# VachaLab/gorder

Measured on AMD Instinct MI355X. Metric: trajectory frames/sec, higher is better.
Workload: dtype f32

## Files before the change

gorder_amd/csrc/gorder_hip.hip:

```cpp
#include <hip/hip_runtime.h>

#include <dlfcn.h>

#include <cmath>
#include <cstdio>
#include <cstdlib>
#include <cstring>
#include <mutex>
#include <new>
#include <string>
#include <deque>
#include <type_traits>
#include <vector>

#include "../../include/gorder_hip.h"
#include "gm_math.h"
#include "plan.h"
#include "collect_store.h"
#include "device_mem.h"
#include "replay_rows.h"
#include "timewise_blocks.h"
#include "ordermap_final.h"
#include "order_route.h"
#include "molecule_rows.h"
// ... 59 lines not shown

struct RepAcc {
    DBuf<u64> acc, rep;
    uint32_t n_rep = 1;
    size_t words = 0;
    bool alloc(size_t n_words, uint32_t n_rep_wanted) {
        words = n_words;
        n_rep = gorder::replica_count(n_rep_wanted, n_words);
        return acc.alloc(words) && rep.alloc((size_t)n_rep * words);
    }
    void reset() { acc.reset(); rep.reset(); words = 0; }
    hipError_t zero_async(hipStream_t stream) {
        const hipError_t e = hipMemsetAsync(acc, 0, words * sizeof(u64), stream);
        return e != hipSuccess ? e : hipMemsetAsync(rep, 0, (size_t)n_rep * words * sizeof(u64), stream);
    }
    hipError_t fold(hipStream_t stream) {
        hipLaunchKernelGGL(k_fold_replicas, dim3((uint32_t)((words + 255) / 256)), dim3(256), 0, stream, acc.get(), rep.get(), n_rep, (uint32_t)words);
        return hipGetLastError();
    }
};

struct gorder_hip_handle {
    void *traj_cache = nullptr;
    void (*traj_cache_free)(gorder_hip_handle *) = nullptr;
    Plan plan;
    gorder_tables_t tables{};
    int device = 0;
    Stream own_stream;
    hipStream_t stream = nullptr;
    DBuf<Tile> d_tiles;
    DBuf<Item> d_items;
    DBuf<uint32_t> d_tile_slots;
    DBuf<DirectItem> d_direct;
    DBuf<Tile> d_ua_tiles;
    DBuf<gorder::UaItem> d_ua_items;
    DBuf<uint32_t> d_ua_tile_slots;
    uint32_t map_nx = 0, map_ny = 0;
    DBuf<u64> d_map_sums, d_map_cnts;
    DBuf<u64> d_map_packed;
    DBuf<u64> d_map_rec;
    DBuf<gorder::MapRun> d_ua_runs, d_runs;
    DBuf<uint32_t> d_ua_run_begin, d_run_begin;
    DBuf<Item> d_items_by_slot;
    DBuf<uint32_t> d_ua_item_run, d_item_run;
    DBuf<uint4> d_lgrid;
    DBuf<LocalRowPre> d_lrowpre;
    DBuf<LocalEdge> d_ledge;
    DBuf<float4> d_lfinfo;
    static constexpr uint32_t kDecidePause = 16;
    DBuf<uint32_t> d_lsummary;
    HBuf<uint32_t> h_lsummary;
    Event lsummary_written;
    bool lsummary_pending = false;
    uint32_t decide_pause = 0;
    uint64_t decide_submits = 0, decide_paused_submits = 0;
    DBuf<uint32_t> d_lneed;
    DBuf<uint2> d_ltodo;
    size_t map_lds_bytes = 0;
    bool map_staged = false;
    uint64_t map_pending = 0;
    uint64_t map_fold_limit = kMapFoldLimit;
    uint32_t map_max_mol = 1;
    DBuf<u64> d_tw_sums, d_tw_cnts;
    uint64_t tw_cap = 0;
    DBuf<u64> d_twx_blocks, d_twx_rows, d_twx_totals, d_twx_edge;
    DBuf<uint32_t> d_twx_groups;
    DBuf<float> d_twx_out;
    DBuf<uint32_t> d_omx_groups;
    DBuf<float> d_omx_out;
    ExtraArgs extra{};
    DBuf<uint32_t> d_geom_group;
    DBuf<float> d_shapes;
    DBuf<float> d_inv_box;
    uint32_t dyn_slab = 4, local_slab = 4;
    bool local_halo = false;
    size_t local_rec_stride = 0;
    DBuf<XtcCheckpoint> d_xtc_cp;
    bool dyn = false;
    DBuf<uint32_t> d_dyn_cloud, d_dyn_heads;
    DBuf<uint32_t> d_dyn_cell_of, d_dyn_count;
    DBuf<float> d_dyn_rec;
    DBuf<float4> d_dyn_normals;
    DBuf<DynCov> d_dyn_cov;
    std::vector<float> last_normals;
    std::vector<float> manual_normals;
    uint32_t manual_frames = 0;
    bool manual_active = false;
    DBuf<uint32_t> d_err;
    u64 *d_acc = nullptr;
    DBuf<u64> own_acc;
    DBuf<u64> d_rep;
    uint32_t n_rep = 32;
    bool rep_dirty = false;
    size_t acc_words = 0;
    DBuf<uint32_t> d_heads, d_membrane, d_methyl_begin, d_methyl_atoms;
    DBuf<uint8_t> d_aflags;
    size_t aflags_rows = 0;
    DBuf<float> d_adist;
    DBuf<float> d_sph_spill, d_sph_stats;
    uint32_t sph_spill = 0, sph_slab = 1u << 20, sph_threads = 1024;
    DBuf<char> d_cl_scratch;
    DBuf<uint32_t> d_cl_head_slot;
    DBuf<uint8_t> d_cl_carry, d_cl_is0;
    DBuf<float> d_cl_stats;
    uint32_t cl_slab = 1, cl_m_max = 0;
    bool cl_stored_w = false;
    bool cl_have_carry = false;
    bool cl_cut = false;
    uint32_t cl_tiles = 0, cl_sort = 0;
    std::vector<uint8_t> cl_is0;
    DBuf<uint32_t> d_lcell_of, d_lcell_count, d_lcell_fill;
    DBuf<float> d_ltrig;
    DBuf<uint32_t> d_arow, d_aframes;
    std::vector<uint32_t> up_arow, up_aframes;
    bool up_arow_valid = false, up_aframes_valid = false;
    bool have_assignment = false;
    uint64_t assignment_frame = 0;
    bool spec_enabled = false;
    DBuf<uint2> d_own;
    DBuf<float4> d_mom;
    DBuf<float> d_head_z;
    DBuf<uint32_t> d_own_head_begin;
    DBuf<uint2> d_own_heads;
    DBuf<float> d_spec_center;
    DBuf<uint8_t> d_spec_ok;
    DBuf<uint32_t> d_spec_counters;
    static constexpr uint32_t kSpecRing = 8;
    HBuf<uint32_t> h_spec_counters;
    Event spec_counters_copied[kSpecRing];
    uint64_t spec_ring_frames[kSpecRing] = {};
    DBuf<uint32_t> d_spec_mol_begin;
    DBuf<SpecSample> d_spec_samples;
    uint64_t spec_batches = 0, spec_fixed = 0, spec_exact_frames = 0;
    DBuf<float> d_stage_xyz[2], d_stage_box[2];
    Event stage_copied[2], stage_computed[2];
    bool stage_used[2] = {false, false};
    int stage_next = 0;
    Stream copy_stream;
    float n2 = 1.0f, n2sq = 1.0f;
    int axis = -1;
    int frames_per_stage = kFramesPerStage;
    bool membrane_is_frame = false;
    bool use_gather = false;
    uint32_t wg_capacity = 256u * 6u;
    uint32_t wg_target = 0;
    uint32_t lw = 0;
    size_t lds_bytes = 0;
    uint64_t n_frames = 0;
    uint64_t err_index = 0;
    std::string err_msg;
    static constexpr uint32_t kTimingEvents = 1024;
    struct TimingSeg { uint32_t label, ev_a, ev_b; };
    bool timing_on = false;
    Event timing_ev[kTimingEvents];
    uint32_t timing_next_ev = 0;
    int timing_open_label = -1;
    uint32_t timing_open_ev = 0;
    std::deque<TimingSeg> timing_pending;
    std::vector<std::string> timing_labels;
    std::vector<double> timing_label_ms;
    std::vector<uint64_t> timing_label_n;
    uint64_t timing_launches = 0;
    std::string timed_kernels;
    std::vector<uint32_t> host_heads, host_dyn_heads;
    DBuf<uint32_t> d_mol_slot0;
    uint64_t err_frame = 0;
// ... 192 lines not shown
        size_t k = 0;
        while (k < h->timing_labels.size() && h->timing_labels[k] != label) k++;
        if (k == h->timing_labels.size()) {
            h->timing_labels.push_back(label);
            h->timing_label_ms.push_back(0.0);
            h->timing_label_n.push_back(0);
            if (!h->timed_kernels.empty()) h->timed_kernels += " + ";
            h->timed_kernels += label;
        }
        h->timing_open_label = (int)k;
        h->timing_open_ev = ev;
    }
    return GORDER_OK;
}
#define TIMING_MARK(h, label)                                   \
    do {                                                        \
        const int tm_ = timing_mark(h, label);                  \
        if (tm_ != GORDER_OK) return tm_;                       \
    } while (0)

bool env_flag(const char *name) {
    const char *v = getenv(name);
    return v && *v && strcmp(v, "0") != 0;
}

int fold_replicas(gorder_hip_handle *h) {
    if (!h->rep_dirty || !h->d_rep) return GORDER_OK;
    const uint32_t n = 4u * h->plan.n_acc;
    hipLaunchKernelGGL(k_fold_replicas, dim3((n + 255) / 256), dim3(256), 0, h->stream, h->d_acc, h->d_rep, h->n_rep, n);
    HIP_TRY(h, hipGetLastError());
    h->rep_dirty = false;
    return GORDER_OK;
}

int fold_maps(gorder_hip_handle *h) {
    if (!h->extra.maps || !h->map_pending) return GORDER_OK;
    const size_t n = (size_t)h->plan.n_acc * h->map_nx * h->map_ny;
    const uint32_t blocks = (uint32_t)std::min<size_t>((n + 255) / 256, 256 * 16);
    hipLaunchKernelGGL(k_fold_maps, dim3(blocks), dim3(256), 0, h->stream, h->d_map_packed, h->d_map_sums, h->d_map_cnts,
                       n, h->tables.leaflets.method != GORDER_LEAFLETS_NONE ? 1 : 0);
    HIP_TRY(h, hipGetLastError());
    h->map_pending = 0;
    return GORDER_OK;
}

int launch_cell_list(gorder_hip_handle *h, const LocalArgs &lo, uint32_t ns, uint32_t n_list, void *counts, size_t count_bytes) {
    const bool three = env_flag("GORDER_HIP_LOCAL_THREE_KERNELS");
    TIMING_MARK(h, n_list <= kLocalBuildMax && !three ? "k_local_build" : "k_local_bin + k_local_scan + k_local_scatter");
    if (n_list <= kLocalBuildMax && !three) {
        if (n_list <= 2u * 8192u) hipLaunchKernelGGL(k_local_build<2>, dim3(ns), dim3(1024), kLocalBuildLds, h->stream, lo);
        else if (n_list <= 5u * 8192u) hipLaunchKernelGGL(k_local_build<5>, dim3(ns), dim3(1024), kLocalBuildLds, h->stream, lo);
        else hipLaunchKernelGGL(k_local_build<kLocalBuildTrips>, dim3(ns), dim3(1024), kLocalBuildLds, h->stream, lo);
        return GORDER_OK;
    }
    HIP_TRY(h, hipMemsetAsync(counts, 0, count_bytes, h->stream));
    const dim3 ga((n_list + 255) / 256, ns);
    hipLaunchKernelGGL(k_local_bin, ga, dim3(256), 0, h->stream, lo);
    hipLaunchKernelGGL(k_local_scan, dim3(ns), dim3(1024), 0, h->stream, lo);
    hipLaunchKernelGGL(k_local_scatter, ga, dim3(256), 0, h->stream, lo);
    return GORDER_OK;
}

int run_dynamic_normals(gorder_hip_handle *h, const FrameArgs &a) {
    int st;
    const uint32_t n_mol = h->plan.n_mol_total;
    if ((st = ensure(h, h->d_dyn_normals, (size_t)a.n_frames * n_mol)) != GORDER_OK) return st;
    const gorder_dynamic_normal_t &dn = h->tables.dynamic_normal;
    const size_t ncell = (size_t)kLocalMaxCells1D * kLocalMaxCells1D;
    LocalArgs lo{};
    lo.xyz = a.xyz; lo.box9 = a.box9; lo.n_atoms = a.n_atoms;
    lo.n_mol_total = n_mol; lo.heads = h->d_dyn_heads; lo.membrane = h->d_dyn_cloud; lo.n_membrane = dn.n_cloud;
    lo.dim = 2; lo.pbc = a.pbc; lo.radius = dn.radius; lo.radius_thr = local_radius_threshold(dn.radius);
    lo.halo = 0; lo.rec_stride = dn.n_cloud;
    lo.cell_of = h->d_dyn_cell_of; lo.trig = h->d_dyn_rec;
    lo.cell_count = h->d_dyn_count; lo.cell_fill = h->d_dyn_count + h->dyn_slab * (ncell + 1);
    lo.err = h->d_err; lo.aframes = nullptr; lo.write_dist_frame = -1;
    for (uint32_t done = 0; done < a.n_frames; done += h->dyn_slab) {
        const uint32_t ns = std::min(a.n_frames - done, h->dyn_slab);
        lo.frame0 = done;
        lo.n_slab = ns;
        if ((st = launch_cell_list(h, lo, ns, dn.n_cloud, h->d_dyn_count,
                                   (size_t)h->dyn_slab * (2 * ncell + 1) * sizeof(uint32_t))) != GORDER_OK) return st;
        TIMING_MARK(h, "k_dyn_cov + k_dyn_eigen");
        hipLaunchKernelGGL(k_dyn_cov, dim3((n_mol + 15) / 16, ns), dim3(256), 0, h->stream, lo, h->d_dyn_cov);
        hipLaunchKernelGGL(k_dyn_eigen, dim3((uint32_t)(((size_t)ns * n_mol + 255) / 256)), dim3(256), 0, h->stream, lo, h->d_dyn_cov,
                           h->d_dyn_normals);
    }
    HIP_TRY(h, hipGetLastError());
    h->last_normals.resize(4 * (size_t)n_mol);
    HIP_TRY(h, hipMemcpyAsync(h->last_normals.data(), h->d_dyn_normals + (size_t)(a.n_frames - 1) * n_mol,
                              4 * sizeof(float) * (size_t)n_mol, hipMemcpyDeviceToHost, h->stream));
    return GORDER_OK;
}

template <int V, int... Vs, class F>
void with_int(int v, F &&f) {
    if constexpr (sizeof...(Vs) > 0) { if (v != V) return with_int<Vs...>(v, f); }
    f(std::integral_constant<int, V>{});
}
template <class F> void with_bool(bool v, F &&f) { if (v) f(std::true_type{}); else f(std::false_type{}); }
template <class F> void with_axis(int axis, F &&f) { with_int<2, 1, 0, -1>(axis, f); }
template <class F> void with_npf(int npf, F &&f) { with_int<4, 5>(npf, f); }
static_assert(gorder::kStageFrames == kRecFrames && gorder::kStageFrames == (uint32_t)kFramesPerStage, "order_route.h: frames of a stage");

int collect_copy_out(gorder_hip_handle *h, gorder::CollectStore &store, const void *d_block, const uint64_t *frames, size_t n_rows);
int launch_molecule_rows(gorder_hip_handle *h, const FrameArgs &a, const gorder::OrderRoute &route) {
    const Plan &p = h->plan;
    const uint32_t n_tiles = (uint32_t)p.tiles.size();
    const bool ac = (h->tables.flags & GORDER_FLAG_TRIG_ACOS_COS) != 0;
    const size_t wpf = (size_t)h->mol.n_groups * p.n_mol_total;
    const uint32_t sub = gorder::molecule_rows_subrange(a.n_frames, wpf, h->mol_stage_bytes);
    int st;
    if ((st = ensure(h, h->d_mol_stage, wpf * sub)) != GORDER_OK) return st;
    MolRowArgs mr{};
    mr.runs = h->d_mol_runs; mr.run_begin = h->d_mol_run_begin; mr.stage = h->d_mol_stage; mr.words_per_frame = (uint32_t)wpf;
    for (uint32_t lo = 0; lo < a.n_frames; lo += sub) {
        const uint32_t hi = std::min(a.n_frames, lo + sub), nf = hi - lo;
        const gorder::FrameChunks c = gorder::extras_chunks(nf, n_tiles, h->wg_target, h->wg_capacity, false, true);
        const uint64_t grid = (uint64_t)n_tiles * c.n_chunks;
        if (grid > 0x7fffffffull) return fail(h, GORDER_ERR_INVALID_ARGUMENT, "batch too large");
        FrameArgs b = a;
        b.frame0 = lo; b.n_frames = hi; b.frames_per_chunk = c.frames_per_chunk;
        TIMING_MARK(h, route.label);
        HIP_TRY(h, hipMemsetAsync(h->d_mol_stage, 0, wpf * nf * sizeof(unsigned long long), h->stream));
        const dim3 g((uint32_t)grid), blk(kBlock);
        with_npf(route.npf, [&](auto NPF) { with_bool(b.pbc, [&](auto PBC) { with_bool(b.leaflets, [&](auto LF) {
            if (ac)
                hipLaunchKernelGGL((k_bonds_tiled_mol<NPF(), true, PBC(), LF(), -1>), g, blk, h->lds_bytes, h->stream, b, mr, b.xyz, b.box9,
                                   b.aflags, b.arow, h->d_tiles, h->d_mol_items, h->d_tile_slots, n_tiles, h->lw);
            else with_int<2, -1>(h->axis, [&](auto AX) {
                hipLaunchKernelGGL((k_bonds_tiled_mol<NPF(), false, PBC(), LF(), AX()>), g, blk, h->lds_bytes, h->stream, b, mr, b.xyz, b.box9,
                                   b.aflags, b.arow, h->d_tiles, h->d_mol_items, h->d_tile_slots, n_tiles, h->lw);
            });
        }); }); });
        HIP_TRY(h, hipGetLastError());
        if ((st = collect_copy_out(h, h->mol_store, h->d_mol_stage, h->mol_frame_index + lo, nf)) != GORDER_OK) return st;
    }
    return GORDER_OK;
}

int launch_orders(gorder_hip_handle *h, FrameArgs &a, const gorder::OrderRoute &route) {
    using gorder::BondFamily, gorder::FrameChunks;
    const Plan &p = h->plan;
    const uint32_t n_tiles = (uint32_t)p.tiles.size();
    const bool ac = (h->tables.flags & GORDER_FLAG_TRIG_ACOS_COS) != 0;
    if (h->dyn && !h->manual_active) {
        ST_TRY(run_dynamic_normals(h, a));
    }
    if (h->extra.geom_kind) {
        int st2;
        if ((st2 = ensure(h, h->d_shapes, (size_t)a.n_frames * 8)) != GORDER_OK) return st2;
        const gorder_geometry_t &ge = h->tables.geometry;
        GeomArgs ga{};
        ga.xyz = a.xyz; ga.box9 = a.box9; ga.n_atoms = a.n_atoms; ga.pbc = a.pbc;
        ga.kind = ge.kind; ga.reference = ge.reference; ga.orientation = ge.orientation;
        for (int d = 0; d < 3; d++) { ga.point[d] = ge.point[d]; ga.structure_box[d] = ge.structure_box[d]; }
        for (int d = 0; d < 2; d++) { ga.xdim[d] = ge.xdim[d]; ga.ydim[d] = ge.ydim[d]; ga.zdim[d] = ge.zdim[d]; ga.span[d] = ge.span[d]; }
        ga.radius = ge.radius; ga.group = h->d_geom_group; ga.n_group = ge.n_group;
        ga.shapes = h->d_shapes; ga.err = h->d_err;
        TIMING_MARK(h, "k_geom_shapes");
        hipLaunchKernelGGL(k_geom_shapes, dim3(a.n_frames), dim3(256), 0, h->stream, ga);
        HIP_TRY(h, hipGetLastError());
    }
    if (route.family == BondFamily::Tiled || route.family == BondFamily::Gather) {
        const FrameChunks c = gorder::tiled_chunks(a.n_frames, (uint32_t)h->frames_per_stage, n_tiles, h->wg_target, h->wg_capacity);
        a.frames_per_chunk = c.frames_per_chunk;
        const uint64_t grid = (uint64_t)n_tiles * c.n_chunks;
        if (grid > 0x7fffffffull) return fail(h, GORDER_ERR_INVALID_ARGUMENT, "batch too large");
        const dim3 g((uint32_t)grid), b(kBlock);
// ... 503 lines not shown
    }
    e.maps = 1; e.plane = om.plane; e.x0 = om.span_x[0]; e.y0 = om.span_y[0];
    e.binx = om.bin[0]; e.biny = om.bin[1]; e.nx = h->map_nx; e.ny = h->map_ny;
    e.inv_binx = 1.0f / om.bin[0]; e.inv_biny = 1.0f / om.bin[1];
    e.bin_core = (om.bin[0] >= 0x1p-40f && om.bin[0] <= 0x1p+40f && om.bin[1] >= 0x1p-40f && om.bin[1] <= 0x1p+40f) ? 1 : 0;
    e.map_packed = h->d_map_packed;
    return GORDER_OK;
}

static int create_geometry(gorder_hip_handle *h, const gorder_tables_t *t) {
    const gorder_geometry_t &ge = t->geometry;
    if (ge.kind == GORDER_GEOM_NONE) return GORDER_OK;
    ExtraArgs &e = h->extra;
    if (ge.kind > GORDER_GEOM_SPHERE || ge.reference > GORDER_GEOMREF_GROUP || ge.orientation > 2)
        return fail(h, GORDER_ERR_INVALID_ARGUMENT, "geometry kind/reference/orientation");
    if (ge.reference == GORDER_GEOMREF_BOX_CENTER && !t->handle_pbc)
        return fail(h, GORDER_ERR_INVALID_ARGUMENT, "box-centre reference needs handle_pbc (pbc.rs:243-245)");
    if (ge.reference == GORDER_GEOMREF_POINT && t->handle_pbc &&
        !(ge.structure_box[0] > 0.0f && ge.structure_box[1] > 0.0f && ge.structure_box[2] > 0.0f))
        return fail(h, GORDER_ERR_INVALID_ARGUMENT, "geometry.structure_box");
    if (ge.reference == GORDER_GEOMREF_GROUP) {
        if (!ge.group || ge.n_group == 0) return fail(h, GORDER_ERR_INVALID_ARGUMENT, "geometry.group");
        std::vector<uint32_t> grp(ge.group, ge.group + ge.n_group);
        for (uint32_t a : grp)
            if (a >= t->n_atoms) return fail(h, GORDER_ERR_INVALID_ARGUMENT, "geometry group index out of range");
        ST_TRY(upload(h, h->d_geom_group, grp));
    }
    e.geom_kind = (int)ge.kind; e.geom_invert = ge.invert ? 1 : 0; e.geom_orient = (int)ge.orientation;
    e.geom_thr = local_radius_threshold(ge.radius);
    h->tables.geometry.group = nullptr;
    return GORDER_OK;
}

static int create_accumulators(gorder_hip_handle *h) {
    const Plan &p = h->plan;
    ST_TRY(allocate(h, h->d_err, kErrWords + 2u));
    HIP_TRY(h, hipMemset(h->d_err, 0xff, kErrWords * sizeof(uint32_t)));
    HIP_TRY(h, hipMemset(h->d_err + kErrWords, 0, 2u * sizeof(uint32_t)));
    h->acc_words = 4 * (size_t)p.n_acc + 1;
    ST_TRY(allocate(h, h->own_acc, h->acc_words, 0));
    h->d_acc = h->own_acc;
    if (const char *e = getenv("GORDER_HIP_MAP_FOLD_LIMIT")) {
        const long v = atol(e);
        if (v >= 2 && (unsigned long long)v <= kMapFoldLimit) h->map_fold_limit = (uint64_t)v;
    }
    if (const char *e = getenv("GORDER_HIP_REPLICAS")) {
        const int r = atoi(e);
        if (r >= 1 && r <= 1024) h->n_rep = (uint32_t)r;
    }
    return p.n_acc ? allocate(h, h->d_rep, (size_t)h->n_rep * 4u * p.n_acc, 0) : GORDER_OK;
}

static int local_build_attributes(gorder_hip_handle *h) {
    for (const void *fn : {reinterpret_cast<const void *>(k_local_build<2>), reinterpret_cast<const void *>(k_local_build<5>),
                           reinterpret_cast<const void *>(k_local_build<kLocalBuildTrips>)})
        HIP_TRY(h, hipFuncSetAttribute(fn, hipFuncAttributeMaxDynamicSharedMemorySize, (int)kLocalBuildLds));
    return GORDER_OK;
}

static int create_dynamic_normals(gorder_hip_handle *h, const gorder_tables_t *t) {
    const gorder_dynamic_normal_t &dn = t->dynamic_normal;
    if (!dn.enabled) return GORDER_OK;
    const Plan &p = h->plan;
    if (!(dn.radius > 0.0f)) return fail(h, GORDER_ERR_INVALID_ARGUMENT, "dynamic normals need a positive radius");
    if (!dn.cloud || dn.n_cloud == 0) return fail(h, GORDER_ERR_INVALID_ARGUMENT, "dynamic normals need the NormalHeads group");
    if (!p.direct.empty()) return fail(h, GORDER_ERR_INVALID_ARGUMENT, "dynamic normals: a bond spans more than the LDS window");
    std::vector<uint32_t> cloud(dn.cloud, dn.cloud + dn.n_cloud), nheads;
    for (uint32_t a : cloud)
        if (a >= t->n_atoms) return fail(h, GORDER_ERR_INVALID_ARGUMENT, "NormalHeads index out of range");
    for (uint32_t m = 0; m < t->n_molecule_types; m++) {
        const gorder_moltype_t &mt = t->molecule_types[m];
        if (!mt.normal_heads) return fail(h, GORDER_ERR_INVALID_ARGUMENT, "dynamic normals need normal_heads[] per molecule type");
        for (uint32_t k = 0; k < mt.n_molecules; k++) {
            if (mt.normal_heads[k] >= t->n_atoms) return fail(h, GORDER_ERR_INVALID_ARGUMENT, "normal head index out of range");
            nheads.push_back(mt.normal_heads[k]);
        }
    }
    ST_TRY(upload(h, h->d_dyn_cloud, cloud));
    ST_TRY(upload(h, h->d_dyn_heads, nheads));
    h->host_dyn_heads = nheads;
    const size_t nm = dn.n_cloud, ncell = (size_t)kLocalMaxCells1D * kLocalMaxCells1D;
    const size_t sl = h->dyn_slab = local_slab_frames(nm);
    ST_TRY(local_build_attributes(h));
    ST_TRY(allocate(h, h->d_dyn_cell_of, sl * nm));
    ST_TRY(allocate(h, h->d_dyn_rec, sl * nm * 4));
    ST_TRY(allocate(h, h->d_dyn_count, sl * (2 * ncell + 1)));
    ST_TRY(allocate(h, h->d_dyn_cov, sl * (size_t)(p.n_mol_total ? p.n_mol_total : 1)));
    h->dyn = true;
    return GORDER_OK;
}

static int create_leaflet_tables(gorder_hip_handle *h, const gorder_tables_t *t, std::vector<uint32_t> &heads) {
    const gorder_leaflets_t &lf = t->leaflets;
    const Plan &p = h->plan;
    if (lf.method > GORDER_LEAFLETS_CLUSTERING) return fail(h, GORDER_ERR_INVALID_ARGUMENT, "leaflets.method");
    if (lf.method != GORDER_LEAFLETS_SPHERICAL && lf.method != GORDER_LEAFLETS_CLUSTERING && lf.normal_dim > 2) return fail(h, GORDER_ERR_INVALID_ARGUMENT, "leaflets.normal_dim");
    std::vector<uint32_t> mb(1, 0), ma;
    for (uint32_t m = 0; m < t->n_molecule_types; m++) {
        const gorder_moltype_t &mt = t->molecule_types[m];
        if (lf.method != GORDER_LEAFLETS_MANUAL && !mt.heads)
            return fail(h, GORDER_ERR_INVALID_ARGUMENT, "leaflets need heads[] per molecule type");
        if (lf.method == GORDER_LEAFLETS_INDIVIDUAL && (!mt.methyls || mt.n_methyls == 0))
            return fail(h, GORDER_ERR_INVALID_ARGUMENT, "individual leaflets need methyls[]");
        for (uint32_t k = 0; k < mt.n_molecules; k++) {
            const uint32_t hd = mt.heads ? mt.heads[k] : 0;
            if (hd >= t->n_atoms) return fail(h, GORDER_ERR_INVALID_ARGUMENT, "head index out of range");
            heads.push_back(hd);
            if (lf.method == GORDER_LEAFLETS_INDIVIDUAL)
                for (uint32_t q = 0; q < mt.n_methyls; q++) {
                    const uint32_t a = mt.methyls[(size_t)k * mt.n_methyls + q];
                    if (a >= t->n_atoms) return fail(h, GORDER_ERR_INVALID_ARGUMENT, "methyl index out of range");
                    ma.push_back(a);
                }
            mb.push_back((uint32_t)ma.size());
        }
    }
    ST_TRY(upload(h, h->d_heads, heads));
    h->host_heads = heads;
    if (lf.method == GORDER_LEAFLETS_LOCAL) {
        std::vector<uint32_t> ms;
        for (uint32_t m = 0; m < t->n_molecule_types; m++) ms.insert(ms.end(), t->molecule_types[m].n_molecules, p.slot0[m]);
        ST_TRY(upload(h, h->d_mol_slot0, ms));
    }
    ST_TRY(upload(h, h->d_methyl_begin, mb));
    ST_TRY(upload(h, h->d_methyl_atoms, ma));
    if (lf.method == GORDER_LEAFLETS_LOCAL && !(lf.radius > 0.0f))
        return fail(h, GORDER_ERR_INVALID_ARGUMENT, "local leaflets need a positive radius");
    if (lf.method == GORDER_LEAFLETS_GLOBAL || lf.method == GORDER_LEAFLETS_LOCAL) {
        if (!lf.membrane || lf.n_membrane == 0)
            return fail(h, GORDER_ERR_INVALID_ARGUMENT, "global/local leaflets need the membrane group");
        std::vector<uint32_t> mem(lf.membrane, lf.membrane + lf.n_membrane);
        for (uint32_t a : mem)
            if (a >= t->n_atoms) return fail(h, GORDER_ERR_INVALID_ARGUMENT, "membrane index out of range");
        ST_TRY(upload(h, h->d_membrane, mem));
        h->membrane_is_frame = lf.n_membrane == t->n_atoms && !env_flag("GORDER_HIP_LEAFLETS_GENERIC");
        for (uint32_t i = 0; i < lf.n_membrane && h->membrane_is_frame; i++) h->membrane_is_frame = mem[i] == i;
    }
    return GORDER_OK;
}

static int upload_cluster_group(gorder_hip_handle *h, const gorder_tables_t *t, const std::vector<uint32_t> &heads, bool ascending,
                                std::vector<uint32_t> &head_slot) {
    const gorder_leaflets_t &lf = t->leaflets;
    std::vector<uint32_t> grp(lf.membrane, lf.membrane + lf.n_membrane);
    std::vector<int32_t> slot_of(t->n_atoms, -1);
    for (uint32_t i = 0; i < lf.n_membrane; i++) {
        if (grp[i] >= t->n_atoms) return fail(h, GORDER_ERR_INVALID_ARGUMENT, "leaflets.membrane: index out of range");
        if (ascending && i && grp[i] <= grp[i - 1]) return fail(h, GORDER_ERR_INVALID_ARGUMENT, "leaflets.membrane: clustering needs ascending, distinct atoms");
        if (slot_of[grp[i]] < 0) slot_of[grp[i]] = (int32_t)i;
    }
    for (uint32_t hd : heads) {
        if (slot_of[hd] < 0)
            return fail(h, GORDER_ERR_INVALID_ARGUMENT, "molecule_types[].heads: a head is not a member of leaflets.membrane");
        head_slot.push_back((uint32_t)slot_of[hd]);
    }
    return upload(h, h->d_membrane, grp);
}

static int create_spherical(gorder_hip_handle *h, const gorder_tables_t *t, const std::vector<uint32_t> &heads) {
    const gorder_leaflets_t &lf = t->leaflets;
    if (!lf.membrane || lf.n_membrane < 2)
        return fail(h, GORDER_ERR_INVALID_ARGUMENT, "leaflets.n_membrane: spherical clustering needs at least two group atoms");
    std::vector<uint32_t> head_slot;
    ST_TRY(upload_cluster_group(h, t, heads, false, head_slot));
    h->sph_threads = lf.n_membrane <= 256u * (uint32_t)kSphKeep ? 256u : 1024u;
    const uint32_t resident = h->sph_threads * (uint32_t)kSphKeep;
// ... 1767 lines not shown
```

gorder_amd/csrc/kernels_normals.h:

```cpp
#pragma once

namespace {

__device__ void sym3_smallest_eigenvector(double a00, double a01, double a02, double a11, double a12, double a22,
                                          double (&out)[3]) {
    double v[3][3] = {{1, 0, 0}, {0, 1, 0}, {0, 0, 1}};
    double a[3][3] = {{a00, a01, a02}, {a01, a11, a12}, {a02, a12, a22}};
    for (int sweep = 0; sweep < 32; sweep++) {
        const double off = a[0][1] * a[0][1] + a[0][2] * a[0][2] + a[1][2] * a[1][2];
        const double dia = a[0][0] * a[0][0] + a[1][1] * a[1][1] + a[2][2] * a[2][2];
        if (!(off > 1e-34 * dia)) break;
#pragma unroll
        for (int p = 0; p < 2; p++)
#pragma unroll
            for (int q = p + 1; q < 3; q++) {
                if (a[p][q] == 0.0) continue;
                const double theta = (a[q][q] - a[p][p]) / (2.0 * a[p][q]);
                const double t = (theta >= 0.0 ? 1.0 : -1.0) / (fabs(theta) + sqrt(theta * theta + 1.0));
                const double c = 1.0 / sqrt(t * t + 1.0), sn = t * c;
                const int r = 3 - p - q;
                const double apq = a[p][q], arp = a[r][p], arq = a[r][q];
                a[p][p] = a[p][p] - t * apq;
                a[q][q] = a[q][q] + t * apq;
                a[p][q] = a[q][p] = 0.0;
// ... 12 lines not shown
    const bool m2 = a[2][2] < d01;
    out[0] = m2 ? v[0][2] : (m1 ? v[0][1] : v[0][0]);
    out[1] = m2 ? v[1][2] : (m1 ? v[1][1] : v[1][0]);
    out[2] = m2 ? v[2][2] : (m1 ? v[2][1] : v[2][0]);
    const double lead = out[2] != 0.0 ? out[2] : (out[1] != 0.0 ? out[1] : out[0]);
    if (lead < 0.0) { out[0] = -out[0]; out[1] = -out[1]; out[2] = -out[2]; }
}

struct DynCov { double n, sx, sy, sz, sxx, sxy, sxz, syy, syz, szz; };

__global__ __launch_bounds__(256) void k_dyn_cov(LocalArgs a, DynCov *__restrict__ cov) {
    const uint32_t lane = threadIdx.x & 63u, row = lane >> 4, sub = lane & 15u;
    const uint32_t m_raw = (blockIdx.x * 4u + (threadIdx.x >> 6)) * 4u + row;
    const uint32_t s = blockIdx.y;
    if ((blockIdx.x * 4u + (threadIdx.x >> 6)) * 4u >= a.n_mol_total) return;
    const bool mol_ok = m_raw < a.n_mol_total;
    const uint32_t m = mol_ok ? m_raw : a.n_mol_total - 1u;
    const uint32_t f = a.aframes ? a.aframes[s] : a.frame0 + s;
    float box[3];
    frame_box(a, f, box);
    uint32_t nca, ncb, ka, kb;
    int da, db;
    local_grid(a, box, nca, ncb, da, db, ka, kb);
    const float *x = a.xyz + (size_t)f * a.n_atoms * 3u;
    const float *hp = x + 3u * (size_t)a.heads[m];
    const float hx = hp[0], hy = hp[1], hz = hp[2];
    const bool undefined = hx != hx;
    int bad = 0;
    uint32_t ha = 0, hb = 0;
    if (a.pbc) {
        const float wa = gm_wrap(hp[da], box[da], bad), wb = gm_wrap(hp[db], box[db], bad);
        ha = (uint32_t)fminf(fmaxf(floorf(wa / box[da] * (float)nca), 0.0f), (float)(nca - 1u));
        hb = (uint32_t)fminf(fmaxf(floorf(wb / box[db] * (float)ncb), 0.0f), (float)(ncb - 1u));
    }
    const uint32_t *cstart = a.cell_count + (size_t)s * (kLocalMaxCells1D * kLocalMaxCells1D + 1u);
    const LocalRec *rec = reinterpret_cast<const LocalRec *>(a.trig) + (size_t)s * a.rec_stride;
    const float thr = a.radius_thr;
    const bool pbc = a.pbc != 0;
    const uint32_t n_rows = 2u * ka + 1u, n_cols = 2u * kb + 1u;
    const uint32_t a0 = (ha + nca - ka) % nca, b0 = (hb + ncb - kb) % ncb;
    const uint32_t b1 = min(b0 + n_cols, ncb), b2 = b0 + n_cols - b1;
    double sx = 0.0, sy = 0.0, sz = 0.0, sxx = 0.0, sxy = 0.0, sxz = 0.0, syy = 0.0, syz = 0.0, szz = 0.0;
    uint32_t cnt = 0;
    auto take = [&](const LocalRec r, bool valid) {
        float dx = r.x - hx, dy = r.y - hy, dz = r.z - hz;
        if (pbc) { dx = gm_min_image(dx, box[0], bad); dy = gm_min_image(dy, box[1], bad); dz = gm_min_image(dz, box[2], bad); }
        if (valid && (dx * dx + dy * dy) + dz * dz < thr) {
            const double ex = (double)dx, ey = (double)dy, ez = (double)dz;
            cnt += 1;
            sx += ex; sy += ey; sz += ez;
            sxx = __builtin_fma(ex, ex, sxx); sxy = __builtin_fma(ex, ey, sxy); sxz = __builtin_fma(ex, ez, sxz);
            syy = __builtin_fma(ey, ey, syy); syz = __builtin_fma(ey, ez, syz); szz = __builtin_fma(ez, ez, szz);
        }
    };
    auto walk = [&](uint32_t q0, uint32_t q1, uint32_t first, uint32_t step) {
        for (uint32_t q = q0 + first; q < q1; q += 4u * step) {
            LocalRec r[4];
#pragma unroll
            for (uint32_t u = 0; u < 4u; u++) r[u] = rec[min(q + u * step, q1 - 1u)];
#pragma unroll
            for (uint32_t u = 0; u < 4u; u++) take(r[u], q + u * step < q1);
        }
    };
    if (!undefined && mol_ok) {
        if (n_rows == 1u && n_cols == 1u) {
            walk(cstart[a0 * ncb + b0], cstart[a0 * ncb + b1], sub, 16u);
        } else if (sub < n_rows) {
            const uint32_t rw = ((a0 + sub) % nca) * ncb;
            walk(cstart[rw + b0], cstart[rw + b1], 0u, 1u);
            if (b2) walk(cstart[rw], cstart[rw + b2], 0u, 1u);
        }
    }
    cnt = row_sum(cnt);
    sx = row_sum(sx); sy = row_sum(sy); sz = row_sum(sz);
    sxx = row_sum(sxx); sxy = row_sum(sxy); sxz = row_sum(sxz);
    syy = row_sum(syy); syz = row_sum(syz); szz = row_sum(szz);
    if (sub == 15u && mol_ok) {
        if (undefined) raise_error(a.err, GORDER_ERR_UNDEFINED_POSITION, f, kStageSystem, 0, 0, m);
        cov[(size_t)s * a.n_mol_total + m] = DynCov{undefined ? -1.0 : (double)cnt, sx, sy, sz, sxx, sxy, sxz, syy, syz, szz};
    }
    if (bad) raise_box_range(a.err, f);
}

__global__ __launch_bounds__(256) void k_dyn_eigen(LocalArgs a, const DynCov *__restrict__ cov, float4 *__restrict__ out) {
    const size_t i = (size_t)blockIdx.x * 256u + threadIdx.x;
    if (i >= (size_t)a.n_slab * a.n_mol_total) return;
    const uint32_t s = (uint32_t)(i / a.n_mol_total), m = (uint32_t)(i - (size_t)s * a.n_mol_total);
    const uint32_t f = a.aframes ? a.aframes[s] : a.frame0 + s;
    const DynCov c = cov[i];
    if (c.n < 0.0) return;
    float4 o = make_float4(__builtin_nanf(""), __builtin_nanf(""), __builtin_nanf(""), (float)c.n);
    if (c.n >= 3.0) {
        const double inv = 1.0 / c.n;
        double e[3];
        sym3_smallest_eigenvector(c.sxx - c.sx * c.sx * inv, c.sxy - c.sx * c.sy * inv, c.sxz - c.sx * c.sz * inv,
                                  c.syy - c.sy * c.sy * inv, c.syz - c.sy * c.sz * inv, c.szz - c.sz * c.sz * inv, e);
        const float fx = (float)e[0], fy = (float)e[1], fz = (float)e[2];
        const float len = __builtin_sqrtf((fx * fx + fy * fy) + fz * fz);
        o.x = fx / len; o.y = fy / len; o.z = fz / len;
    }
    out[(size_t)f * a.n_mol_total + m] = o;
}

}
```

Before: 20.61 million.

## Fuse dynamic-normal covariance and eigen kernels into one LDS-staged per-frame kernel

```diff
diff --git a/gorder_amd/csrc/gorder_hip.hip b/gorder_amd/csrc/gorder_hip.hip
--- a/gorder_amd/csrc/gorder_hip.hip
+++ b/gorder_amd/csrc/gorder_hip.hip
@@ -165,6 +165,8 @@
     DBuf<float> d_dyn_rec;
     DBuf<float4> d_dyn_normals;
     DBuf<DynCov> d_dyn_cov;
+    bool dyn_lanes = true;
+    uint32_t dyn_lds_bytes = kDynLanesLds;
     std::vector<float> last_normals;
     std::vector<float> manual_normals;
     uint32_t manual_frames = 0;
@@ -523,9 +525,14 @@
         if ((st = launch_cell_list(h, lo, ns, dn.n_cloud, h->d_dyn_count,
                                    (size_t)h->dyn_slab * (2 * ncell + 1) * sizeof(uint32_t))) != GORDER_OK) return st;
         TIMING_MARK(h, "k_dyn_cov + k_dyn_eigen");
-        hipLaunchKernelGGL(k_dyn_cov, dim3((n_mol + 15) / 16, ns), dim3(256), 0, h->stream, lo, h->d_dyn_cov);
-        hipLaunchKernelGGL(k_dyn_eigen, dim3((uint32_t)(((size_t)ns * n_mol + 255) / 256)), dim3(256), 0, h->stream, lo, h->d_dyn_cov,
-                           h->d_dyn_normals);
+        if (h->dyn_lanes && dn.n_cloud <= kLocalBuildMax && !env_flag("GORDER_HIP_LOCAL_THREE_KERNELS")) {
+            hipLaunchKernelGGL(k_dyn_lanes, dim3(ns), dim3(kDynLanesBlock), h->dyn_lds_bytes, h->stream, lo, h->dyn_lds_bytes,
+                               h->d_dyn_normals);
+        } else {
+            hipLaunchKernelGGL(k_dyn_cov, dim3((n_mol + 15) / 16, ns), dim3(256), 0, h->stream, lo, h->d_dyn_cov);
+            hipLaunchKernelGGL(k_dyn_eigen, dim3((uint32_t)(((size_t)ns * n_mol + 255) / 256)), dim3(256), 0, h->stream, lo, h->d_dyn_cov,
+                               h->d_dyn_normals);
+        }
     }
     HIP_TRY(h, hipGetLastError());
     h->last_normals.resize(4 * (size_t)n_mol);
@@ -1195,6 +1202,12 @@
     const size_t nm = dn.n_cloud, ncell = (size_t)kLocalMaxCells1D * kLocalMaxCells1D;
     const size_t sl = h->dyn_slab = local_slab_frames(nm);
     ST_TRY(local_build_attributes(h));
+    h->dyn_lanes = !env_flag("GORDER_HIP_DYN_ROWS");
+    if (const char *e = getenv("GORDER_HIP_DYN_LDS_BYTES")) {
+        const long long v = atoll(e);
+        if (v >= 0 && v < (long long)kDynLanesLds) h->dyn_lds_bytes = (uint32_t)v;
+    }
+    HIP_TRY(h, hipFuncSetAttribute(reinterpret_cast<const void *>(k_dyn_lanes), hipFuncAttributeMaxDynamicSharedMemorySize, (int)kDynLanesLds));
     ST_TRY(allocate(h, h->d_dyn_cell_of, sl * nm));
     ST_TRY(allocate(h, h->d_dyn_rec, sl * nm * 4));
     ST_TRY(allocate(h, h->d_dyn_count, sl * (2 * ncell + 1)));
diff --git a/gorder_amd/csrc/kernels_normals.h b/gorder_amd/csrc/kernels_normals.h
--- a/gorder_amd/csrc/kernels_normals.h
+++ b/gorder_amd/csrc/kernels_normals.h
@@ -118,13 +118,7 @@
     if (bad) raise_box_range(a.err, f);
 }
 
-__global__ __launch_bounds__(256) void k_dyn_eigen(LocalArgs a, const DynCov *__restrict__ cov, float4 *__restrict__ out) {
-    const size_t i = (size_t)blockIdx.x * 256u + threadIdx.x;
-    if (i >= (size_t)a.n_slab * a.n_mol_total) return;
-    const uint32_t s = (uint32_t)(i / a.n_mol_total), m = (uint32_t)(i - (size_t)s * a.n_mol_total);
-    const uint32_t f = a.aframes ? a.aframes[s] : a.frame0 + s;
-    const DynCov c = cov[i];
-    if (c.n < 0.0) return;
+__device__ __forceinline__ float4 dyn_normal(const DynCov &c) {
     float4 o = make_float4(__builtin_nanf(""), __builtin_nanf(""), __builtin_nanf(""), (float)c.n);
     if (c.n >= 3.0) {
         const double inv = 1.0 / c.n;
@@ -135,7 +129,111 @@
         const float len = __builtin_sqrtf((fx * fx + fy * fy) + fz * fz);
         o.x = fx / len; o.y = fy / len; o.z = fz / len;
     }
-    out[(size_t)f * a.n_mol_total + m] = o;
-}
-
-}
+    return o;
+}
+
+__global__ __launch_bounds__(256) void k_dyn_eigen(LocalArgs a, const DynCov *__restrict__ cov, float4 *__restrict__ out) {
+    const size_t i = (size_t)blockIdx.x * 256u + threadIdx.x;
+    if (i >= (size_t)a.n_slab * a.n_mol_total) return;
+    const uint32_t s = (uint32_t)(i / a.n_mol_total), m = (uint32_t)(i - (size_t)s * a.n_mol_total);
+    const uint32_t f = a.aframes ? a.aframes[s] : a.frame0 + s;
+    const DynCov c = cov[i];
+    if (c.n < 0.0) return;
+    out[(size_t)f * a.n_mol_total + m] = dyn_normal(c);
+}
+
+constexpr uint32_t kDynLanesBlock = 1024;
+constexpr uint32_t kDynLanesLds = 80u * 1024u;
+struct DynRecLds { const float4 *p; __device__ __forceinline__ LocalRec operator()(uint32_t q) const { const float4 v = p[q]; return LocalRec{v.x, v.y, v.z}; } };
+struct DynRecMem { const LocalRec *p; __device__ __forceinline__ LocalRec operator()(uint32_t q) const { return p[q]; } };
+
+template <typename Rec>
+__device__ __forceinline__ void dyn_lanes_frame(const LocalArgs &a, uint32_t f, const float *box, uint32_t nca, uint32_t ncb,
+                                                int da, int db, uint32_t ka, uint32_t kb, const uint32_t *cstart, Rec rec,
+                                                float4 *__restrict__ out) {
+    const float *x = a.xyz + (size_t)f * a.n_atoms * 3u;
+    const float thr = a.radius_thr;
+    const bool pbc = a.pbc != 0;
+    const uint32_t n_rows = 2u * ka + 1u, n_cols = 2u * kb + 1u;
+    int bad = 0;
+    for (uint32_t m = threadIdx.x; m < a.n_mol_total; m += kDynLanesBlock) {
+        const float *hp = x + 3u * (size_t)a.heads[m];
+        const float hx = hp[0], hy = hp[1], hz = hp[2];
+        if (hx != hx) {
+            raise_error(a.err, GORDER_ERR_UNDEFINED_POSITION, f, kStageSystem, 0, 0, m);
+            continue;
+        }
+        uint32_t ha = 0, hb = 0;
+        if (pbc) {
+            const float wa = gm_wrap(hp[da], box[da], bad), wb = gm_wrap(hp[db], box[db], bad);
+            ha = (uint32_t)fminf(fmaxf(floorf(wa / box[da] * (float)nca), 0.0f), (float)(nca - 1u));
+            hb = (uint32_t)fminf(fmaxf(floorf(wb / box[db] * (float)ncb), 0.0f), (float)(ncb - 1u));
+        }
+        uint32_t a0 = ha + nca - ka, b0 = hb + ncb - kb;
+        a0 -= a0 >= nca ? nca : 0u;
+        b0 -= b0 >= ncb ? ncb : 0u;
+        const uint32_t b1 = min(b0 + n_cols, ncb), b2 = b0 + n_cols - b1;
+        double sx = 0.0, sy = 0.0, sz = 0.0, sxx = 0.0, sxy = 0.0, sxz = 0.0, syy = 0.0, syz = 0.0, szz = 0.0;
+        uint32_t cnt = 0;
+        auto take = [&](const LocalRec r) {
+            float dx = r.x - hx, dy = r.y - hy, dz = r.z - hz;
+            if (pbc) {
+                bool slow = false;
+                const float mx = gm_min_image_step(dx, box[0], slow), my = gm_min_image_step(dy, box[1], slow),
+                            mz = gm_min_image_step(dz, box[2], slow);
+                if (__builtin_expect(slow, 0)) {
+                    dx = gm_min_image_loop(dx, box[0], bad); dy = gm_min_image_loop(dy, box[1], bad); dz = gm_min_image_loop(dz, box[2], bad);
+                } else {
+                    dx = mx; dy = my; dz = mz;
+                }
+            }
+            if ((dx * dx + dy * dy) + dz * dz < thr) {
+                const double ex = (double)dx, ey = (double)dy, ez = (double)dz;
+                cnt += 1;
+                sx += ex; sy += ey; sz += ez;
+                sxx = __builtin_fma(ex, ex, sxx); sxy = __builtin_fma(ex, ey, sxy); sxz = __builtin_fma(ex, ez, sxz);
+                syy = __builtin_fma(ey, ey, syy); syz = __builtin_fma(ey, ez, syz); szz = __builtin_fma(ez, ez, szz);
+            }
+        };
+        auto run_of = [&](uint32_t k, uint32_t &q, uint32_t &qe) {
+            uint32_t ra = a0 + (k >> 1);
+            ra -= ra >= nca ? nca : 0u;
+            const uint32_t rw = ra * ncb;
+            q = cstart[(k & 1u) ? rw : rw + b0];
+            qe = cstart[(k & 1u) ? rw + b2 : rw + b1];
+        };
+        const uint32_t k_end = 2u * n_rows, k_step = b2 ? 1u : 2u;
+        for (uint32_t k = 0; k < k_end; k += k_step) {
+            uint32_t q, qe;
+            run_of(k, q, qe);
+            for (; q < qe; q++) take(rec(q));
+        }
+        out[(size_t)f * a.n_mol_total + m] = dyn_normal(DynCov{(double)cnt, sx, sy, sz, sxx, sxy, sxz, syy, syz, szz});
+    }
+    if (bad) raise_box_range(a.err, f);
+}
+
+__global__ __launch_bounds__(kDynLanesBlock, 8) void k_dyn_lanes(LocalArgs a, uint32_t lds_bytes, float4 *__restrict__ out) {
+    extern __shared__ float4 l_dyn[];
+    const uint32_t s = blockIdx.x;
+    const uint32_t f = a.aframes ? a.aframes[s] : a.frame0 + s;
+    float box[3];
+    frame_box(a, f, box);
+    uint32_t nca, ncb, ka, kb;
+    int da, db;
+    local_grid(a, box, nca, ncb, da, db, ka, kb);
+    const uint32_t *cstart = a.cell_count + (size_t)s * (kLocalMaxCells1D * kLocalMaxCells1D + 1u);
+    const LocalRec *rec = reinterpret_cast<const LocalRec *>(a.trig) + (size_t)s * a.rec_stride;
+    const uint32_t n_rec = a.n_membrane, n_start = nca * ncb + 1u;
+    if ((size_t)n_rec * sizeof(float4) + (size_t)n_start * sizeof(uint32_t) <= lds_bytes) {
+        uint32_t *l_start = reinterpret_cast<uint32_t *>(l_dyn + n_rec);
+        for (uint32_t i = threadIdx.x; i < n_rec; i += kDynLanesBlock) { const LocalRec r = rec[i]; l_dyn[i] = make_float4(r.x, r.y, r.z, 0.0f); }
+        for (uint32_t i = threadIdx.x; i < n_start; i += kDynLanesBlock) l_start[i] = cstart[i];
+        __syncthreads();
+        dyn_lanes_frame(a, f, box, nca, ncb, da, db, ka, kb, l_start, DynRecLds{l_dyn}, out);
+    } else {
+        dyn_lanes_frame(a, f, box, nca, ncb, da, db, ka, kb, cstart, DynRecMem{rec}, out);
+    }
+}
+
+}
```

Measured after the change: 20.89 million (median of 3 runs). No clear change (+1.4%).
